# yaricom/Plastic-UNet

Hardware: AMD Instinct MI355X
Metric: training images/sec (128x128, bs=32 per GPU) (higher is better)
Workload: dtype f32; 1 GPU; C2: UNetp depth 5 base_ch 64, oja rule, 1x128x128, fwd+BCE+bwd+Adam; global_batch=32, per_gpu_batch=32, img=128, parallelism=single, step_launch=eager

## Files before the change

### include/plastic_unet.h

```cpp
#ifndef PLASTIC_UNET_H
#define PLASTIC_UNET_H

#include <stddef.h>
#include <stdint.h>

#ifdef __cplusplus
extern "C" {
#endif

#define PU_ABI_VERSION 3

typedef enum {
    PU_OK = 0,
    PU_ERR_INVALID = -1,
    PU_ERR_UNSUPPORTED = -2,
    PU_ERR_LAUNCH = -3,
    PU_ERR_WORKSPACE = -4
} pu_status;

int pu_abi_version(void);
const char* pu_last_error(void);
const char* pu_build_id(void);
int pu_device_info(int device, int* num_cu, int* clock_khz, long long* hbm_bytes);

enum { PU_EPI_RELU = 1, PU_EPI_ACCUM = 2, PU_EPI_SHUFFLE2 = 4, PU_EPI_RESID = 8, PU_CONV_NO_HALO = 16,
       PU_CONV_HALO_V1 = 32, PU_CONV_NO_SMALLX6 = 64, PU_CONV_HALO_DMA = 128, PU_EPI_OUT_BF16 = 256 };

typedef struct {
    int batch;
    int in_h, in_w;
    int out_h, out_w;
    int kh, kw, stride, pad;
    const float* src0; int c0;
    const float* src1; int c1;
    const float* weight; int k_pad; int cgroup;
    int n;
    const float* bias;
    float* dst0; int n0;
    float* dst1;
    const float* mask0;
    const float* mask1;
    int flags;
    void* workspace; size_t ws_bytes;
    const float* resid;
    int shuf_h, shuf_w, shuf_off;
    const void* weight6;
    const void* wino;
    const float* chan_scale; int chan_scale_ld;
} pu_conv_args;

int pu_conv_igemm(const pu_conv_args* a, void* stream);
typedef struct {
    const float* w;
    void* out;
    int cout, cin;
    int dgrad;
} pu_wino_job;
size_t pu_wino_bytes(int n, int c);
int pu_pack_wino(const pu_wino_job* jobs, int n_jobs, void* stream);
int pu_split_weight6(const float* packed, void* out, int n, int k_pad, void* stream);
size_t pu_conv_igemm_workspace_bytes(const pu_conv_args* a);
int pu_conv_igemm_tile(const pu_conv_args* a, int* bm, int* bn, int* mode, int* ksplit);

typedef struct {
    int batch;
    int in_h, in_w;
    int out_h, out_w;
    int kh, kw, stride, pad;
    const float* rows; int n;
    const float* src0; int c0;
    const float* src1; int c1;
    int bias_mode;
    float* dweight;
    float* dbias;
    int accumulate;
    int math;
} pu_wgrad_args;

size_t pu_wgrad_workspace_bytes(const pu_wgrad_args* a);
// ... 175 lines not shown
```

### plastic-unet_amd/csrc/igemm.hip

```cpp
#include "conv_common.h"
#include <type_traits>

namespace pu {


constexpr int IG_BK = 16;
constexpr int IG_LDS = IG_BK + 4;

enum { LOAD_CHUNK16 = 0, LOAD_VEC4 = 1, LOAD_SCALAR = 2 };


template <int MODE>
__device__ __forceinline__ f32x4 load_a4(const IgemmParams& p, int pb, int hb, int wb, int k) {
    f32x4 v = {0.f, 0.f, 0.f, 0.f};
    if (MODE == LOAD_SCALAR) {
#pragma unroll
        for (int e = 0; e < 4; ++e) {
            int ke = k + e;
            if (ke < p.K) {
                int tap = fdiv(ke, p.dC);
                int c = ke - tap * p.C;
                int r = fdiv(tap, p.dKw);
                int s = tap - r * p.kw;
                int hi = hb + r, wi = wb + s;
// ... 882 lines not shown
                xb[i] = *reinterpret_cast<const f32x4*>(a + (a_row0 + i * 32) * 16 + pos1);
            }
#pragma unroll
            for (int pl = 0; pl < 3; ++pl)
#pragma unroll
                for (int j = 0; j < FN; ++j)
                    fw[pl][j] = *reinterpret_cast<const bf16x8_t*>(wp + ((pl * 2 + lh) * BN + b_row0 + j * 32) * 4);
#pragma unroll
            for (int i = 0; i < FM; ++i) {
                bf16x8_t xh, xm, xl;
                split3_pairs(xa[i], xb[i], xh, xm, xl);
#pragma unroll
                for (int j = 0; j < FN; ++j) {
                    f32x16 c = acc[i][j];
                    c = __builtin_amdgcn_mfma_f32_32x32x16_bf16(fw[1][j], xm, c, 0, 0, 0);
                    c = __builtin_amdgcn_mfma_f32_32x32x16_bf16(fw[2][j], xh, c, 0, 0, 0);
                    c = __builtin_amdgcn_mfma_f32_32x32x16_bf16(fw[0][j], xl, c, 0, 0, 0);
                    c = __builtin_amdgcn_mfma_f32_32x32x16_bf16(fw[1][j], xh, c, 0, 0, 0);
                    c = __builtin_amdgcn_mfma_f32_32x32x16_bf16(fw[0][j], xm, c, 0, 0, 0);
                    c = __builtin_amdgcn_mfma_f32_32x32x16_bf16(fw[0][j], xh, c, 0, 0, 0);
                    acc[i][j] = c;
                }
                if (i == 0) {
                    if constexpr (u + 2 < SPG) issue(g, std::integral_constant<int, u + 2>{});
                    else issue(g + 1, std::integral_constant<int, u + 2 - SPG>{});
                }
            }
        });
    }
    asm volatile("s_waitcnt vmcnt(0)" ::: "memory");
    if (p.ksplit == 1) {
        epilogue<BM, BN, WM, WN, true>(p, acc, m_blk, n_blk, wm, wn, lr, lh);
        return;
    }
    float* part = p.part + (long long)kz * p.M * p.N;
#pragma unroll
    for (int i = 0; i < FM; ++i) {
        const int m = m_blk + wm * (BM / WM) + i * 32 + lr;
        if (m >= p.M) continue;
#pragma unroll
        for (int j = 0; j < FN; ++j)
#pragma unroll
            for (int q = 0; q < 4; ++q) {
                const int n = n_blk + wn * (BN / WN) + j * 32 + 8 * q + 4 * lh;
                if (n >= p.N) continue;
                f32x4 v;
#pragma unroll
                for (int e = 0; e < 4; ++e) v[e] = acc[i][j][4 * q + e];
                *reinterpret_cast<f32x4*>(part + (long long)m * p.N + n) = v;
            }
    }
}

__global__ void split_weight6_kernel(const float* __restrict__ w, __bf16* __restrict__ out, int n, int k_pad) {
#pragma clang fp contract(off)
    const long long total = (long long)n * k_pad;
    for (long long idx = blockIdx.x * 256LL + threadIdx.x; idx < total; idx += (long long)gridDim.x * 256) {
        const int row = (int)(idx / k_pad);
        const int k = (int)(idx - (long long)row * k_pad);
        const float x = w[idx];
        const __bf16 a = (__bf16)x;
        const float r = x - (float)a;
        const __bf16 b = (__bf16)r;
        const __bf16 c = (__bf16)(r - (float)b);
        const int t = k >> 4, half = (k >> 3) & 1, e = k & 7;
        const __bf16 v[3] = {a, b, c};
#pragma unroll
        for (int pl = 0; pl < 3; ++pl)
            out[(((long long)t * 6 + pl * 2 + half) * n + row) * 8 + e] = v[pl];
    }
}

__global__ __launch_bounds__(256) void igemm_splitk_epilogue_kernel(const IgemmParams p) {
    const int nq = p.N >> 2;
    const long long idx = (long long)blockIdx.x * 256 + threadIdx.x;
    if (idx >= (long long)p.M * nq) return;
    const int m = (int)(idx / nq);
    const int n = (int)(idx - (long long)m * nq) * 4;
    const long long mn = (long long)p.M * p.N;
    const float* src = p.part + (long long)m * p.N + n;
    f32x4 v = *reinterpret_cast<const f32x4*>(src);
    for (int z = 1; z < p.ksplit; ++z) v += *reinterpret_cast<const f32x4*>(src + z * mn);
    epi_store4(p, epi_row(p, m), n, v);
}

constexpr int SC_TH = 16, SC_TW = 32;

template <int C, int N, int KP = (9 * C + 15) / 16 * 16>
__global__ __launch_bounds__(256) void smallconv_kernel(const IgemmParams p) {
    constexpr int HH = SC_TH + 2, HWD = SC_TW + 2;
    constexpr int CP = (C + 3) & ~3;
    __shared__ __attribute__((aligned(16))) float tile[HH * HWD * CP];
    const int tiles_w = (p.Wo + SC_TW - 1) / SC_TW;
    const int tiles_h = (p.Ho + SC_TH - 1) / SC_TH;
    int blk = blockIdx.x;
    const int txi = blk % tiles_w;
    blk /= tiles_w;
    const int tyi = blk % tiles_h;
    const int b = blk / tiles_h;
    const int y0 = tyi * SC_TH - 1, x0 = txi * SC_TW - 1;
    const long long img = (long long)b * p.Hi * p.Wi;

    if (C % 4 == 0 && p.c0 % 4 == 0) {
        constexpr int Q = C / 4 > 0 ? C / 4 : 1;
        constexpr int NE = HH * HWD * Q;
        constexpr int PT = (NE + 255) / 256;
// ... 154 lines not shown
            typedef __bf16 bf16x4_t __attribute__((ext_vector_type(4)));
            bf16x4_t o;
#pragma unroll
            for (int e = 0; e < 4; ++e) o[e] = (__bf16)v[e];
            *reinterpret_cast<bf16x4_t*>(reinterpret_cast<__bf16*>(p.dst0) + (long long)m * N + 4 * lane_c) = o;
        } else if (plain) {
            if (p.bias) v += bias4;
            if (p.flags & PU_EPI_RELU) {
#pragma unroll
                for (int e = 0; e < 4; ++e) v[e] = fmaxf(v[e], 0.f);
            }
            *reinterpret_cast<f32x4*>(p.dst0 + (long long)m * N + 4 * lane_c) = v;
        } else {
            epi_store4(p, epi_row(p, m), 4 * lane_c, v);
        }
    }
}

template <int BM, int BN, int WM, int WN>
static void launch_mode(int mode, const IgemmParams& p, dim3 grid, hipStream_t s) {
    switch (mode) {
        case LOAD_CHUNK16: hipLaunchKernelGGL((igemm_kernel<BM, BN, WM, WN, LOAD_CHUNK16>), grid, dim3(256), 0, s, p); break;
        case LOAD_VEC4: hipLaunchKernelGGL((igemm_kernel<BM, BN, WM, WN, LOAD_VEC4>), grid, dim3(256), 0, s, p); break;
        default: hipLaunchKernelGGL((igemm_kernel<BM, BN, WM, WN, LOAD_SCALAR>), grid, dim3(256), 0, s, p); break;
    }
}

static int choose_mode(int c0, int c1) {
    if (c0 % 16 == 0 && c1 % 16 == 0) return LOAD_CHUNK16;
    if (c0 % 4 == 0 && c1 % 4 == 0) return LOAD_VEC4;
    return LOAD_SCALAR;
}

static bool vec_epilogue(const pu_conv_args* a) {
    const bool shuffle = a->flags & PU_EPI_SHUFFLE2;
    const int n0 = shuffle ? a->n : a->n0;
    const uintptr_t al = (uintptr_t)a->dst0 | (uintptr_t)a->dst1 | (uintptr_t)a->mask0 | (uintptr_t)a->mask1 |
                         (uintptr_t)a->bias | ((a->flags & PU_EPI_RESID) ? (uintptr_t)a->resid : 0);
    return (a->n % 4 == 0) && (n0 % 4 == 0) && (al & 15) == 0 && (!shuffle || (a->n / 4) % 4 == 0);
}

static bool uses_x6(const pu_conv_args* a);
static bool lean_ok(const pu_conv_args* a) {
    if (!uses_x6(a)) return false;
    const int C = a->c0 + a->c1;
    if (a->kh != 3 || a->kw != 3 || !(a->cgroup == 16 || a->cgroup == 32)) return false;
    if (a->c1 != 0 && a->c1 != a->c0) return false;
    if (a->k_pad != 9 * C) return false;
    const long long shift = (long long)a->pad * a->in_w + a->pad;
    if (((long long)a->batch * a->in_h * a->in_w + shift) * a->c0 * 4 >= (1LL << 31)) return false;
    if ((long long)a->k_pad * a->n * 12 >= (1LL << 31)) return false;
    return true;
}
static void plan_tiles(const pu_conv_args* a, long long M, int* bm, int* bn, int* ksplit, int* t_per) {
    const int N = a->n;
    const int T = a->k_pad / IG_BK;
    if (!uses_x6(a)) {
        choose_tile(M, N, bm, bn);
        *ksplit = 1;
        *t_per = T;
        if (choose_mode(a->c0, a->c1) == LOAD_CHUNK16 && vec_epilogue(a))
            plan_split(a->k_pad, IG_BK, 8, M, N, *bm, *bn, ksplit, t_per);
        return;
    }
    int target = 512;
    if (N <= 32 && lean_ok(a)) {
        *bn = 32;
        *bm = blocks_for(M, N, 256, 32) >= 480 ? 256 : 128;
    } else if (N <= 64) {
        *bn = 64;
        *bm = blocks_for(M, N, 256, 64) >= 480 ? 256 : 128;
    } else if (a->k_pad >= 2048) {
        *bn = 128;
        *bm = 256;
        target = 256;
    } else {
        *bn = 128;
        *bm = 128;
    }
    *ksplit = 1;
    *t_per = T;
    const int tiles = blocks_for(M, N, *bm, *bn);
    if (tiles >= target - target / 16 || !vec_epilogue(a)) return;
    int ks = ceil_div(target, tiles);
    if (ks > T / 8) ks = T / 8;
    if (ks < 2) return;
    *t_per = ceil_div(T, ks);
    if (lean_ok(a)) {
        const int spg = 9 * (a->cgroup / 16);
        *t_per = ceil_div(*t_per, spg) * spg;
    }
    *ksplit = ceil_div(T, *t_per);
}

static bool conv1x1_small_ok(const pu_conv_args* a) {
    const int C = a->c0 + a->c1;
    return (C == 4 || C == 8) && (a->n == 8 || a->n == 16) && a->kh == 1 && a->kw == 1 && a->stride == 1 &&
           a->pad == 0 && a->in_h == a->out_h && a->in_w == a->out_w && !(a->flags & PU_EPI_SHUFFLE2) &&
           vec_epilogue(a) && a->c0 % 4 == 0 && a->c1 % 4 == 0 && (a->cgroup == 0 || a->cgroup >= C);
}

static bool small_conv_ok(const pu_conv_args* a) {
    const int C = a->c0 + a->c1;
    const bool cset = C == 1 || C == 4 || C == 8 || C == 12 || C == 16;
    const bool nset = a->n == 4 || a->n == 8 || a->n == 16;
    const bool nc = (a->n == 4) ? (C == 4 || C == 8 || C == 16) : true;
    return cset && nset && nc && a->kh == 3 && a->kw == 3 && a->stride == 1 && a->pad == 1 &&
           a->in_h == a->out_h && a->in_w == a->out_w && !(a->flags & PU_EPI_SHUFFLE2) && vec_epilogue(a) &&
           (a->cgroup == 0 || a->cgroup >= C) && (C == 1 || (a->c0 % 4 == 0 && a->c1 % 4 == 0)) &&
           a->k_pad == (9 * C + 15) / 16 * 16;
}

static bool stem_conv_ok(const pu_conv_args* a) {
    const int C = a->c0 + a->c1;
    return C == 1 && a->c1 == 0 && (a->n == 8 || a->n == 16 || a->n == 32 || a->n == 64) && a->kh == 3 && a->kw == 3 && a->stride == 1 &&
           a->pad == 1 && a->in_h == a->out_h && a->in_w == a->out_w && !(a->flags & PU_EPI_SHUFFLE2) &&
           vec_epilogue(a) && (a->cgroup == 0 || a->cgroup >= C);
}

static bool uses_x6(const pu_conv_args* a) {
    return a->weight6 && choose_mode(a->c0, a->c1) == LOAD_CHUNK16 && !small_conv_ok(a);
}

enum { CK_STEM, CK_1X1, CK_SMALLX6, CK_DIRECT, CK_WINO, CK_X6_LEAN, CK_X6, CK_DMA, CK_LOADER };
struct ConvPlan {
    int kind, bm, bn;
    int mode;
    int ksplit, t_per;
    size_t ws_bytes;
};

static ConvPlan plan_conv(const pu_conv_args* a, long long M) {
    ConvPlan pl;
    pl.bn = a->n;
    pl.ksplit = 1;
    pl.t_per = a->k_pad / IG_BK;
    pl.ws_bytes = 0;
    const bool vec = vec_epilogue(a);
    if (stem_conv_ok(a)) {
        pl.kind = CK_STEM;
        pl.mode = 5;
        pl.bm = ST_TH * ST_TW;
        return pl;
    }
    if (conv1x1_small_ok(a)) {
        pl.kind = CK_1X1;
        pl.mode = 3;
        pl.bm = 256;
        return pl;
    }
    if (smallx6_ok(a, vec)) {
        pl.kind = CK_SMALLX6;
        pl.mode = 7;
        pl.bm = a->stride == 2 ? 128 : a->kh == 2 ? 256 : 512;
        return pl;
    }
    if (small_conv_ok(a)) {
        pl.kind = CK_DIRECT;
        pl.mode = 3;
        pl.bm = SC_TH * SC_TW;
        return pl;
    }
    if (wino_ok(a, vec)) {
        pl.kind = CK_WINO;
        pl.mode = 6;
        pl.bn = wino_item_channels(a);
        pl.bm = pl.bn == 64 ? 256 : 128;
        pl.ws_bytes = wino_workspace_bytes(a);
        if (pl.ws_bytes) pl.ksplit = (int)(pl.ws_bytes / ((size_t)M * a->n * sizeof(float)));
    } else {
        plan_tiles(a, M, &pl.bm, &pl.bn, &pl.ksplit, &pl.t_per);
        const int loader = choose_mode(a->c0, a->c1);
        pl.kind = uses_x6(a) ? (lean_ok(a) ? CK_X6_LEAN : CK_X6) : loader == LOAD_CHUNK16 ? CK_DMA : CK_LOADER;
        pl.mode = uses_x6(a) ? 4 : loader;
        if (pl.ksplit > 1) pl.ws_bytes = (size_t)pl.ksplit * (size_t)M * (size_t)a->n * sizeof(float);
    }
    if (pl.ksplit > 1 && (!a->workspace || a->ws_bytes < pl.ws_bytes)) {
        pl.ksplit = 1;
        pl.t_per = a->k_pad / IG_BK;
    }
    return pl;
}

}

using namespace pu;

extern "C" int pu_conv_igemm(const pu_conv_args* a, void* stream) {
    PU_REQUIRE(a != nullptr, "pu_conv_igemm: null args");
    PU_REQUIRE(a->batch > 0 && a->in_h > 0 && a->in_w > 0 && a->out_h > 0 && a->out_w > 0,
               "pu_conv_igemm: bad grid %dx%dx%d -> %dx%d", a->batch, a->in_h, a->in_w, a->out_h, a->out_w);
    PU_REQUIRE(a->kh > 0 && a->kw > 0 && a->stride > 0 && a->pad >= 0, "pu_conv_igemm: bad taps");
    PU_REQUIRE(a->kh * a->kw <= 32, "pu_conv_igemm: at most 32 taps");
    PU_REQUIRE(a->src0 && a->c0 > 0, "pu_conv_igemm: src0 missing");
    PU_REQUIRE(a->c1 == 0 || a->src1, "pu_conv_igemm: src1 missing for c1=%d", a->c1);
    PU_REQUIRE(a->weight && a->dst0 && a->n > 0, "pu_conv_igemm: weight/dst0/n");
    const int C = a->c0 + a->c1;
    const int K = a->kh * a->kw * C;
    PU_REQUIRE(a->k_pad >= K && a->k_pad % IG_BK == 0, "pu_conv_igemm: k_pad %d must be >= %d and a multiple of 16", a->k_pad, K);
    const bool shuffle = a->flags & PU_EPI_SHUFFLE2;
    if (a->flags & PU_EPI_RESID) {
        PU_REQUIRE(a->resid && !shuffle && (a->n0 == a->n), "pu_conv_igemm: RESID needs resid, a single destination, no SHUFFLE2");
    }
    if (shuffle) {
        PU_REQUIRE(a->n % 4 == 0, "pu_conv_igemm: SHUFFLE2 needs n %% 4 == 0");
        PU_REQUIRE(a->shuf_off >= 0 && a->shuf_h >= 0 && a->shuf_w >= 0, "pu_conv_igemm: shuffle geometry");
    } else {
        PU_REQUIRE(a->n0 > 0 && a->n0 <= a->n, "pu_conv_igemm: n0 %d out of range", a->n0);
        PU_REQUIRE(a->n0 == a->n || a->dst1, "pu_conv_igemm: dst1 missing");
    }
    const long long M = (long long)a->batch * a->out_h * a->out_w;
    PU_REQUIRE(M < (1LL << 31) && (long long)a->batch * a->in_h * a->in_w < (1LL << 31), "pu_conv_igemm: too many pixels");

    IgemmParams p;
    p.M = (int)M; p.N = a->n; p.K = K; p.k_pad = a->k_pad;
    p.Hi = a->in_h; p.Wi = a->in_w; p.Ho = a->out_h; p.Wo = a->out_w;
    p.kh = a->kh; p.kw = a->kw; p.stride = a->stride; p.pad = a->pad;
    p.C = C; p.c0 = a->c0; p.c1 = a->c1;
    p.src0 = a->src0; p.src1 = a->src1; p.wt = a->weight; p.bias = a->bias;
    p.dst0 = a->dst0; p.dst1 = a->dst1; p.mask0 = a->mask0; p.mask1 = a->mask1;
    p.n0 = shuffle ? a->n : a->n0; p.flags = a->flags;
    p.resid = (a->flags & PU_EPI_RESID) ? a->resid : nullptr;
    p.shuf_h = a->shuf_h ? a->shuf_h : 2 * a->out_h;
    p.shuf_w = a->shuf_w ? a->shuf_w : 2 * a->out_w;
    p.shuf_off = a->shuf_off;
    p.dWo = make_fastdiv(a->out_w); p.dHo = make_fastdiv(a->out_h);
    p.dC = make_fastdiv(C); p.dKw = make_fastdiv(a->kw); p.dCo = make_fastdiv(shuffle ? a->n / 4 : 1);
    p.taps = a->kh * a->kw;
    p.dTaps = make_fastdiv(p.taps);
    p.cgroup = a->cgroup;
    p.vec_epi = vec_epilogue(a);
    p.in_pix = a->batch * a->in_h * a->in_w;
    p.cscale = a->chan_scale;
    p.cs_ld = a->chan_scale_ld ? a->chan_scale_ld : (shuffle ? a->n / 4 : a->n);
    p.dHW = make_fastdiv(a->out_h * a->out_w);
    if (a->chan_scale) {
        PU_REQUIRE(((uintptr_t)a->chan_scale & 15) == 0 && p.cs_ld % 4 == 0 && p.cs_ld >= (shuffle ? a->n / 4 : a->n),
                   "pu_conv_igemm: chan_scale must be 16-byte aligned with a row stride >= its channels and %% 4 == 0 (ld %d)", p.cs_ld);
    }

    const int mode = choose_mode(a->c0, a->c1);
    PU_REQUIRE(a->cgroup == 0 || a->cgroup == 16 || a->cgroup == 32, "pu_conv_igemm: cgroup %d", a->cgroup);
    PU_REQUIRE(a->cgroup == 0 || (mode == LOAD_CHUNK16 && a->c0 % a->cgroup == 0 && a->c1 % a->cgroup == 0),
               "pu_conv_igemm: cgroup %d needs channel counts (%d, %d) that are multiples of it", a->cgroup, a->c0, a->c1);
    if (mode != LOAD_SCALAR) {
        PU_REQUIRE(((uintptr_t)a->src0 & 15) == 0 && ((uintptr_t)a->src1 & 15) == 0,
                   "pu_conv_igemm: sources must be 16-byte aligned");
    }
    PU_REQUIRE(((uintptr_t)a->weight & 15) == 0, "pu_conv_igemm: weight must be 16-byte aligned");

    const bool out_bf16 = a->flags & PU_EPI_OUT_BF16;
    if (out_bf16) {
        PU_REQUIRE(stem_conv_ok(a) && !a->mask0 && !a->mask1 && !a->resid && !a->chan_scale && a->n0 == a->n &&
                       !(a->flags & (PU_EPI_ACCUM | PU_EPI_SHUFFLE2)) && ((uintptr_t)a->dst0 & 7) == 0,
                   "pu_conv_igemm: PU_EPI_OUT_BF16 is the single-channel stem conv only (c0 1, 3x3/s1/p1, n 8/16/32/64, "
                   "no mask/resid/accum/shuffle/chan_scale, 8-byte aligned dst0)");
    }
    const ConvPlan pl = plan_conv(a, M);
    if (pl.kind == CK_WINO || pl.kind == CK_X6_LEAN || pl.kind == CK_X6) {
        PU_REQUIRE(((uintptr_t)a->weight6 & 15) == 0, "pu_conv_igemm: weight6 must be 16-byte aligned");
    }
    hipStream_t s = as_stream(stream);
    const int N = a->n;
    const int bm = pl.bm, bn = pl.bn;
    p.ksplit = pl.ksplit;
    p.t_per = pl.t_per;
    p.part = (float*)a->workspace;
    p.gn = ceil_div(N, bn);
    const dim3 grid(ceil_div(M, bm) * p.gn * p.ksplit);
    const char* what = "pu_conv_igemm";
    switch (pl.kind) {
        case CK_STEM: {
            const dim3 sgrid((unsigned)(((a->out_w + ST_TW - 1) / ST_TW) * ((a->out_h + ST_TH - 1) / ST_TH) * a->batch));
            if (out_bf16) {
                if (N == 64) hipLaunchKernelGGL((stem_conv_kernel<64, true>), sgrid, dim3(256), 0, s, p);
                else if (N == 32) hipLaunchKernelGGL((stem_conv_kernel<32, true>), sgrid, dim3(256), 0, s, p);
                else if (N == 16) hipLaunchKernelGGL((stem_conv_kernel<16, true>), sgrid, dim3(256), 0, s, p);
                else hipLaunchKernelGGL((stem_conv_kernel<8, true>), sgrid, dim3(256), 0, s, p);
                what = "pu_conv_igemm (stem, bf16 out)";
                break;
            }
            if (N == 64) hipLaunchKernelGGL((stem_conv_kernel<64>), sgrid, dim3(256), 0, s, p);
            else if (N == 32) hipLaunchKernelGGL((stem_conv_kernel<32>), sgrid, dim3(256), 0, s, p);
            else if (N == 16) hipLaunchKernelGGL((stem_conv_kernel<16>), sgrid, dim3(256), 0, s, p);
            else hipLaunchKernelGGL((stem_conv_kernel<8>), sgrid, dim3(256), 0, s, p);
            what = "pu_conv_igemm (stem)";
            break;
        }
        case CK_1X1: {
            const dim3 g1((unsigned)(M / 256 + 1 < 8192 ? M / 256 + 1 : 8192));
            if (C == 4 && N == 8) hipLaunchKernelGGL((conv1x1_small_kernel<4, 8>), g1, dim3(256), 0, s, p);
            else if (C == 4) hipLaunchKernelGGL((conv1x1_small_kernel<4, 16>), g1, dim3(256), 0, s, p);
            else if (N == 8) hipLaunchKernelGGL((conv1x1_small_kernel<8, 8>), g1, dim3(256), 0, s, p);
            else hipLaunchKernelGGL((conv1x1_small_kernel<8, 16>), g1, dim3(256), 0, s, p);
            what = "pu_conv_igemm (1x1 small-channel)";
            break;
        }
        case CK_SMALLX6:
            return smallx6_launch(a, p, s);
        case CK_DIRECT: {
            const dim3 sgrid((unsigned)(((a->out_w + SC_TW - 1) / SC_TW) * ((a->out_h + SC_TH - 1) / SC_TH) * a->batch));
#define PU_SC(C_, N_) if (C == C_ && N == N_) hipLaunchKernelGGL((smallconv_kernel<C_, N_>), sgrid, dim3(256), 0, s, p)
            PU_SC(1, 8); else PU_SC(1, 16); else PU_SC(4, 8); else PU_SC(4, 16); else PU_SC(8, 8); else PU_SC(8, 16);
            else PU_SC(12, 8); else PU_SC(12, 16); else PU_SC(16, 8); else PU_SC(16, 16);
            else PU_SC(4, 4); else PU_SC(8, 4); else PU_SC(16, 4);
#undef PU_SC
            what = "pu_conv_igemm (small-channel)";
            break;
        }
        case CK_WINO:
            p.gn = N / 64;
            wino_launch(a, p, s);
            what = "pu_conv_igemm (winograd x6)";
            break;
        case CK_X6_LEAN: {
            p.wt = reinterpret_cast<const float*>(a->weight6);
            const int cg = a->cgroup / 16;
#define PU_XL(BM_, BN_, WM_, WN_, NW_)                                                                          \
    do {                                                                                                        \
        if (cg == 2) hipLaunchKernelGGL((igemm_x6_lean_kernel<BM_, BN_, WM_, WN_, NW_, 2>), grid, dim3(NW_ * 64), 0, s, p); \
        else hipLaunchKernelGGL((igemm_x6_lean_kernel<BM_, BN_, WM_, WN_, NW_, 1>), grid, dim3(NW_ * 64), 0, s, p); \
    } while (0)
            if (bm == 256 && bn == 128) PU_XL(256, 128, 8, 1, 8);
            else if (bm == 256 && bn == 64) PU_XL(256, 64, 8, 1, 8);
            else if (bm == 128 && bn == 128) PU_XL(128, 128, 4, 1, 4);
            else if (bm == 128 && bn == 64) PU_XL(128, 64, 2, 2, 4);
            else if (bm == 256) PU_XL(256, 32, 4, 1, 4);
            else PU_XL(128, 32, 4, 1, 4);
#undef PU_XL
            what = "pu_conv_igemm (x6 lean)";
            break;
        }
        case CK_X6:
            p.wt = reinterpret_cast<const float*>(a->weight6);
#define PU_X6(BM_, BN_, WM_, WN_) hipLaunchKernelGGL((igemm_x6_kernel<BM_, BN_, WM_, WN_>), grid, dim3(256), 0, s, p)
            if (bm == 256 && bn == 128)
                hipLaunchKernelGGL((igemm_x6_kernel<256, 128, 8, 1, 8>), grid, dim3(512), 0, s, p);
            else if (bm == 256) PU_X6(256, 64, 4, 1);
            else if (bm == 128 && bn == 128) PU_X6(128, 128, 4, 1);
            else PU_X6(128, 64, 2, 2);
#undef PU_X6
            break;
        case CK_DMA:
            if (bm == 256) hipLaunchKernelGGL((igemm_dma_kernel<256, 64, 4, 1, 3>), grid, dim3(256), 0, s, p);
            else if (bm == 128 && bn == 128) hipLaunchKernelGGL((igemm_dma_kernel<128, 128, 2, 2, 3>), grid, dim3(256), 0, s, p);
            else if (bm == 128) hipLaunchKernelGGL((igemm_dma_kernel<128, 64, 2, 2, 3>), grid, dim3(256), 0, s, p);
            else hipLaunchKernelGGL((igemm_dma_kernel<64, 64, 2, 2, 3>), grid, dim3(256), 0, s, p);
            break;
        default:
            if (bm == 256) launch_mode<256, 64, 4, 1>(pl.mode, p, grid, s);
            else if (bm == 128 && bn == 128) launch_mode<128, 128, 2, 2>(pl.mode, p, grid, s);
            else if (bm == 128) launch_mode<128, 64, 2, 2>(pl.mode, p, grid, s);
            else launch_mode<64, 64, 2, 2>(pl.mode, p, grid, s);
    }
    if (p.ksplit > 1) {
        const long long threads = M * (N / 4);
        hipLaunchKernelGGL(igemm_splitk_epilogue_kernel, dim3((unsigned)((threads + 255) / 256)), dim3(256), 0, s, p);
    }
    return check_launch(what);
}

extern "C" int pu_split_weight6(const float* packed, void* out, int n, int k_pad, void* stream) {
    PU_REQUIRE(packed && out && n > 0 && k_pad > 0 && k_pad % IG_BK == 0, "pu_split_weight6: bad args");
    const long long total = (long long)n * k_pad;
    long long blocks = (total + 255) / 256;
    if (blocks > 4096) blocks = 4096;
    hipLaunchKernelGGL(split_weight6_kernel, dim3((unsigned)blocks), dim3(256), 0, as_stream(stream), packed,
                       (__bf16*)out, n, k_pad);
    return check_launch("pu_split_weight6");
}

extern "C" size_t pu_conv_igemm_workspace_bytes(const pu_conv_args* a) {
    if (!a || a->batch <= 0 || a->out_h <= 0 || a->out_w <= 0 || a->n <= 0 || a->k_pad <= 0) return 0;
    return plan_conv(a, (long long)a->batch * a->out_h * a->out_w).ws_bytes;
}

extern "C" int pu_conv_igemm_tile(const pu_conv_args* a, int* bm, int* bn, int* mode, int* ksplit) {
    PU_REQUIRE(a && bm && bn && mode, "pu_conv_igemm_tile: null args");
    const ConvPlan pl = plan_conv(a, (long long)a->batch * a->out_h * a->out_w);
    *bm = pl.bm;
    *bn = pl.bn;
    *mode = pl.mode;
    if (ksplit) *ksplit = pl.ksplit;
    return PU_OK;
}
// ... 1 lines not shown
```

### plastic-unet_amd/punet/_lib.py

```python
import ctypes
import os

HERE = os.path.dirname(os.path.abspath(__file__))
LIB_PATH = os.environ.get("PLASTIC_UNET_LIB",
                          os.path.join(os.path.dirname(HERE), "lib", "libplastic_unet.so"))

c_int, c_ll, c_size, c_float, c_void_p = ctypes.c_int, ctypes.c_longlong, ctypes.c_size_t, ctypes.c_float, ctypes.c_void_p
c_double = ctypes.c_double
P = ctypes.c_void_p

(PU_EPI_RELU, PU_EPI_ACCUM, PU_EPI_SHUFFLE2, PU_EPI_RESID, PU_CONV_NO_HALO, PU_CONV_HALO_V1, PU_CONV_NO_SMALLX6,
 PU_CONV_HALO_DMA, PU_EPI_OUT_BF16) = 1, 2, 4, 8, 16, 32, 64, 128, 256
PU_PACK_CONV_FWD, PU_PACK_CONV_DGRAD, PU_PACK_CONVT_FWD, PU_PACK_CONVT_DGRAD, PU_PACK_CONVT3_FWD = 0, 1, 2, 3, 4
PU_RULE_HEBB, PU_RULE_OJA = 0, 1


ABI_VERSION = 3


class ConvArgs(ctypes.Structure):
    _fields_ = [("batch", c_int), ("in_h", c_int), ("in_w", c_int), ("out_h", c_int), ("out_w", c_int),
                ("kh", c_int), ("kw", c_int), ("stride", c_int), ("pad", c_int),
                ("src0", P), ("c0", c_int), ("src1", P), ("c1", c_int),
                ("weight", P), ("k_pad", c_int), ("cgroup", c_int), ("n", c_int), ("bias", P),
                ("dst0", P), ("n0", c_int), ("dst1", P), ("mask0", P), ("mask1", P), ("flags", c_int),
                ("workspace", P), ("ws_bytes", c_size),
                ("resid", P), ("shuf_h", c_int), ("shuf_w", c_int), ("shuf_off", c_int),
                ("weight6", P), ("wino", P), ("chan_scale", P), ("chan_scale_ld", c_int)]


class WgradArgs(ctypes.Structure):
    _fields_ = [("batch", c_int), ("in_h", c_int), ("in_w", c_int), ("out_h", c_int), ("out_w", c_int),
                ("kh", c_int), ("kw", c_int), ("stride", c_int), ("pad", c_int),
                ("rows", P), ("n", c_int), ("src0", P), ("c0", c_int), ("src1", P), ("c1", c_int),
                ("bias_mode", c_int), ("dweight", P), ("dbias", P), ("accumulate", c_int),
                ("math", c_int)]


class PlasticArgs(ctypes.Structure):
    _fields_ = [("batch", c_int), ("nbf", c_int), ("x", P), ("hebb", P), ("w", P), ("alpha", P), ("eta", P),
                ("y", P), ("hebb_out", P), ("rule", c_int)]


class PlasticHeadArgs(ctypes.Structure):
    _fields_ = [("batch", c_int), ("nbf", c_int), ("channels", c_int), ("feat", P), ("feat_bf16", c_int),
                ("out_w", P), ("out_b", P), ("hebb", P), ("w", P), ("alpha", P), ("eta", P), ("x", P), ("y", P),
                ("hebb_out", P), ("rule", c_int)]


class PlasticBwdArgs(ctypes.Structure):
    _fields_ = [("batch", c_int), ("nbf", c_int), ("x", P), ("hebb", P), ("w", P), ("alpha", P), ("y", P),
                ("dy", P), ("dx", P), ("dw", P), ("dalpha", P)]


class PlasticBwdTraceArgs(ctypes.Structure):
    _fields_ = [("batch", c_int), ("nbf", c_int), ("rule", c_int), ("x", P), ("hebb", P), ("w", P), ("alpha", P),
                ("eta", P), ("y", P), ("dy", P), ("dhebb_out", P), ("dx", P), ("dw", P), ("dalpha", P), ("dhebb", P),
                ("deta", P)]


class AdamTensor(ctypes.Structure):
    _fields_ = [("param", P), ("grad", P), ("exp_avg", P), ("exp_avg_sq", P), ("numel", c_ll)]


class WinoJob(ctypes.Structure):
# ... 111 lines not shown
```

### plastic-unet_amd/punet/kernels.py

```python
import ctypes
import os

import torch

from . import _lib
from ._lib import (ConvArgs, WgradArgs, PlasticArgs, PlasticHeadArgs, PlasticBwdArgs, PlasticBwdTraceArgs, AdamTensor,
                   PackJob, WinoJob, check,
                   PU_EPI_RELU, PU_EPI_ACCUM, PU_EPI_SHUFFLE2, PU_EPI_RESID, PU_CONV_NO_HALO, PU_CONV_HALO_V1,
                   PU_CONV_NO_SMALLX6, PU_EPI_OUT_BF16)

__all__ = ["KernelProfiler", "igemm", "wgrad", "pack_weight", "nchw_to_nhwc", "maxpool2_fwd", "maxpool2_bwd",
           "outconv_fwd", "outconv_bwd", "plastic_fwd", "trace_update", "plastic_bwd", "plastic_bwd_trace", "bce_fwd",
           "bce_bwd", "adam_multi", "pack_weights", "round16", "cgroup_for", "device_info", "lib"]


def lib():
    return _lib.load()


_PROF = None
_MODES = {0: "chunk16", 1: "vec4", 2: "scalar", 3: "direct", 4: "x6", 5: "stem", 6: "wino", 7: "x6s"}

_FP32_MATH = os.environ.get("PU_FP32_MATH", "split6")


_CONV_HALO = os.environ.get("PU_CONV_HALO", "1") != "0"


def set_conv_halo(on):
    global _CONV_HALO
    if isinstance(on, str) or on not in (0, 1):
        raise ValueError("set_conv_halo: 1 / True (halo and rows) or 0 / False (per-tap), not %r" % (on,))
    prev, _CONV_HALO = int(_CONV_HALO), bool(on)
    return prev


def _halo_flags():
    return 0 if _CONV_HALO else PU_CONV_NO_HALO


def fp32_math():
    return _FP32_MATH


_WINO = os.environ.get("PU_WINO", "1") != "0"


_SMALLX6 = os.environ.get("PU_SMALLX6", "1") != "0"


def set_smallx6(on):
    global _SMALLX6
    prev, _SMALLX6 = _SMALLX6, bool(on)
    return prev


def set_wino(on):
    global _WINO
    prev, _WINO = _WINO, bool(on)
    return prev


def wino_wanted(w, mode):
    if mode not in (0, 1) or w.dim() != 4 or w.shape[2:] != (3, 3) or _FP32_MATH != "split6":
        return False
    n, c = (w.shape[0], w.shape[1]) if mode == 0 else (w.shape[1], w.shape[0])
    return c % 32 == 0 and n % 64 == 0 and (c >= 128 or n <= 64 or n % 128 == 0)


def pack_wino(jobs):
    if not jobs:
        return
    arr = (WinoJob * len(jobs))()
    nbytes = 0.0
    for i, (w, out, dgrad) in enumerate(jobs):
        _req(w, "w")
        arr[i] = WinoJob(w.data_ptr(), out.data_ptr(), w.shape[0], w.shape[1], int(dgrad))
        nbytes += 4.0 * w.numel() + 2.0 * out.numel()
    with _Rec("pack_wino", nbytes=nbytes):
        check(lib().pu_pack_wino(arr, len(jobs), _stream()), "pu_pack_wino")


def set_fp32_math(mode):
    global _FP32_MATH
    if mode not in ("split6", "native"):
        raise ValueError("fp32 math must be 'split6' or 'native', got %r" % (mode,))
    prev, _FP32_MATH = _FP32_MATH, mode
    return prev


class KernelProfiler:

    def __init__(self):
        self.records = []

    def __enter__(self):
        global _PROF
        self._prev, _PROF = _PROF, self
        return self

    def __exit__(self, *exc):
# ... 47 lines not shown
    return torch.cuda.current_stream().cuda_stream


def round16(k):
    return (k + 15) // 16 * 16


def _req(t, name, dtype=torch.float32):
    if t is None:
        return
    if not t.is_cuda:
        raise RuntimeError("%s must be on the ROCm device (got %s); the plastic U-Net path has no CPU "
                           "fallback" % (name, t.device))
    if t.dtype != dtype:
        raise RuntimeError("%s must be %s (got %s)" % (name, dtype, t.dtype))
    if not t.is_contiguous():
        raise RuntimeError("%s must be contiguous" % name)


BF16 = torch.bfloat16


def _act_dtype(t):
    return BF16 if t.dtype == BF16 else torch.float32


def device_info(device=0):
    L = lib()
    cu, clk, mem = ctypes.c_int(), ctypes.c_int(), ctypes.c_longlong()
    check(L.pu_device_info(device, ctypes.byref(cu), ctypes.byref(clk), ctypes.byref(mem)), "pu_device_info")
    return cu.value, clk.value, mem.value


def cgroup_for(c0, c1=0):
    if c0 % 32 == 0 and c1 % 32 == 0:
        return 32
    if c0 % 16 == 0 and c1 % 16 == 0:
        return 16
    return 0


def igemm(*, batch, in_hw, out_hw, k, stride, pad, src0, c0, weight, k_pad, n, dst0, n0=None,
          src1=None, c1=0, bias=None, dst1=None, mask0=None, mask1=None, relu=False, accum=False,
          shuffle=False, cgroup=0, resid=None, shuf=(0, 0, 0), chan_scale=None):
    dt = _act_dtype(src0)
    out_bf16 = dt == torch.float32 and dst0 is not None and dst0.dtype == BF16
    for t, nm in ((src0, "src0"), (src1, "src1"), (weight, "weight"), (dst0, "dst0"),
                  (dst1, "dst1"), (mask0, "mask0"), (mask1, "mask1"), (resid, "resid")):
        _req(t, nm, BF16 if (out_bf16 and nm == "dst0") else dt)
    _req(bias, "bias")
    _req(chan_scale, "chan_scale")
    flags = (PU_EPI_RELU if relu else 0) | (PU_EPI_ACCUM if accum else 0) | (PU_EPI_SHUFFLE2 if shuffle else 0) \
        | (PU_EPI_RESID if resid is not None else 0) | _halo_flags() | (0 if _SMALLX6 else PU_CONV_NO_SMALLX6) \
        | (PU_EPI_OUT_BF16 if out_bf16 else 0)
    a = ConvArgs(batch, in_hw[0], in_hw[1], out_hw[0], out_hw[1], k, k, stride, pad,
                 _p(src0), c0, _p(src1), c1, _p(weight), k_pad, cgroup, n, _p(bias),
                 _p(dst0), n if n0 is None else n0, _p(dst1), _p(mask0), _p(mask1), flags, None, 0,
                 _p(resid), shuf[0], shuf[1], shuf[2])
    if chan_scale is not None:
        if chan_scale.dim() != 2 or chan_scale.shape[0] != batch:
            raise RuntimeError("chan_scale must be [batch, channels]")
        a.chan_scale, a.chan_scale_ld = chan_scale.data_ptr(), chan_scale.shape[1]
    w6 = getattr(weight, "_split6", None) if (dt != BF16 and _FP32_MATH == "split6") else None
    wn = getattr(weight, "_wino", None) if (w6 is not None and _WINO) else None
    if w6 is not None:
        a.weight6 = w6.data_ptr()
    if wn is not None:
        a.wino = wn.data_ptr()
        key = (batch, tuple(in_hw), tuple(out_hw), k, stride, pad, c0, c1, n, a.n0, k_pad, cgroup, flags,
               tuple(None if t is None else t.data_ptr() % 16
                     for t in (src0, src1, bias, dst0, dst1, mask0, mask1, resid, chan_scale, weight, w6, wn)))
        _ensure_direct(a, weight, key)
    elif getattr(weight, "_direct_ok", True) is False:
        _refresh_direct(weight)
    L = lib()
    if dt == BF16:
        _igemm_bf16(L, a, batch, out_hw, k, c0, c1, n, dst0)
        return
    nbytes = L.pu_conv_igemm_workspace_bytes(ctypes.byref(a))
    if nbytes:
        ws = torch.empty(nbytes // 4 + 1, dtype=torch.float32, device=dst0.device)
        a.workspace, a.ws_bytes = ws.data_ptr(), nbytes
    if _PROF is None:
        check(L.pu_conv_igemm(ctypes.byref(a), _stream()), "pu_conv_igemm")
        return
    bm, bn, mode, ks = ctypes.c_int(), ctypes.c_int(), ctypes.c_int(), ctypes.c_int()
    L.pu_conv_igemm_tile(ctypes.byref(a), ctypes.byref(bm), ctypes.byref(bn), ctypes.byref(mode), ctypes.byref(ks))
    M = batch * out_hw[0] * out_hw[1]
    tag = "igemm<%dx%d,%s%s>" % (bm.value, bn.value, _MODES[mode.value], ",k%d" % ks.value if ks.value > 1 else "")
    nb = 0.0
    if mode.value in (3, 5, 7):
        per = (c0 + c1) + n * (1 + int(accum) + int(resid is not None)) + n0_mask(n, n0, mask0, mask1)
        nb = 4.0 * M * per
    with _Rec(tag, flops=2.0 * M * n * k * k * (c0 + c1), nbytes=nb):
        check(L.pu_conv_igemm(ctypes.byref(a), _stream()), "pu_conv_igemm")


def n0_mask(n, n0, mask0, mask1):
    n0 = n if n0 is None else n0
    return (n0 if mask0 is not None else 0) + (n - n0 if mask1 is not None else 0)


def _igemm_bf16(L, a, batch, out_hw, k, c0, c1, n, dst0):
    nbytes = L.pu_conv_igemm_bf16_workspace_bytes(ctypes.byref(a))
    if nbytes:
        ws = torch.empty(nbytes // 4 + 1, dtype=torch.float32, device=dst0.device)
        a.workspace, a.ws_bytes = ws.data_ptr(), nbytes
# ... 449 lines not shown
```

Baseline: 4723 images/s.

## Add lean direct-to-LDS x6 kernel for 1x1 and 2x2-stride-2 convolutions

Adds a new split-bf16 (x6) implicit-GEMM kernel for pointwise 1x1 and 2x2 stride-2 convolutions. It uses buffer loads straight into LDS, a triple-buffered stage ring, and precomputed per-lane offsets. Before this, those shapes fell to the generic x6 kernel with its heavier loader. The aim is to cut address arithmetic and overlap global loads with MFMA work. The path is on by default and can be disabled by an environment variable or flag; it adds a new code path with its own tile-selection and bounds checks.

```diff
diff --git a/include/plastic_unet.h b/include/plastic_unet.h
--- a/include/plastic_unet.h
+++ b/include/plastic_unet.h
@@ -24,7 +24,8 @@
 int pu_device_info(int device, int* num_cu, int* clock_khz, long long* hbm_bytes);
 
 enum { PU_EPI_RELU = 1, PU_EPI_ACCUM = 2, PU_EPI_SHUFFLE2 = 4, PU_EPI_RESID = 8, PU_CONV_NO_HALO = 16,
-       PU_CONV_HALO_V1 = 32, PU_CONV_NO_SMALLX6 = 64, PU_CONV_HALO_DMA = 128, PU_EPI_OUT_BF16 = 256 };
+       PU_CONV_HALO_V1 = 32, PU_CONV_NO_SMALLX6 = 64, PU_CONV_HALO_DMA = 128, PU_EPI_OUT_BF16 = 256,
+       PU_CONV_NO_POINT_LEAN = 512 };
 
 typedef struct {
     int batch;
diff --git a/plastic-unet_amd/csrc/igemm.hip b/plastic-unet_amd/csrc/igemm.hip
--- a/plastic-unet_amd/csrc/igemm.hip
+++ b/plastic-unet_amd/csrc/igemm.hip
@@ -958,6 +958,181 @@
     }
 }
 
+template <int BM, int BN, int WM, int WN, int NW, int TAPS, int CG>
+__global__ __launch_bounds__(NW * 64) void igemm_x6_point_kernel(const IgemmParams p) {
+    constexpr int FM = BM / WM / 32;
+    constexpr int FN = BN / WN / 32;
+    constexpr int A_LD = BM / (16 * NW);
+    constexpr int W_TOT = 6 * BN / 64;
+    constexpr int W_LD = (W_TOT + NW - 1) / NW;
+    constexpr bool SINK = (W_TOT % NW) != 0;
+    constexpr int G = A_LD + W_LD;
+    constexpr int A_FL = BM * 16;
+    constexpr int W_FL = BN * 6 * 4;
+    constexpr int STAGE = A_FL + W_FL;
+    static_assert(WM * WN == NW && A_LD >= 1 && (TAPS == 1 || TAPS == 4) && (CG == 1 || CG == 2), "point tile");
+
+    __shared__ __attribute__((aligned(16))) float lds[3 * STAGE + (SINK ? 256 : 0)];
+
+    const int tid = threadIdx.x;
+    const int lane = tid & 63;
+    const int wave = __builtin_amdgcn_readfirstlane(tid >> 6);
+    const int wm = wave % WM, wn = wave / WM;
+    const int lr = lane & 31, lh = lane >> 5;
+    int tile = xcd_remap(blockIdx.x, gridDim.x);
+    const int kz = tile / (gridDim.x / p.ksplit);
+    tile -= kz * (gridDim.x / p.ksplit);
+    const int mb = tile / p.gn;
+    const int m_blk = mb * BM;
+    const int n_blk = (tile - mb * p.gn) * BN;
+
+    const int cs = p.c0;
+    const unsigned a_bytes = (unsigned)((long long)p.in_pix * cs * 4);
+    const unsigned w_bytes = (unsigned)((long long)p.k_pad * p.N * 6);
+
+    const int lq = lane >> 2;
+    const int kc = (lane & 3) ^ ((lane >> 4) & 3);
+    unsigned vo[A_LD];
+#pragma unroll
+    for (int j = 0; j < A_LD; ++j) {
+        const int m = m_blk + wave * (BM / NW) + 16 * j + lq;
+        unsigned o = LEAN_OOB;
+        if (m < p.M) {
+            int pix = m;
+            if constexpr (TAPS == 4) {
+                const int t = fdiv(m, p.dWo);
+                const int wo = m - t * p.Wo;
+                const int b = fdiv(t, p.dHo);
+                const int ho = t - b * p.Ho;
+                pix = (b * p.Hi + 2 * ho) * p.Wi + 2 * wo;
+            }
+            o = (unsigned)pix * (unsigned)(cs * 4) + kc * 16;
+        }
+        vo[j] = o;
+    }
+    unsigned wv[W_LD];
+#pragma unroll
+    for (int j = 0; j < W_LD; ++j) {
+        const int I = wave + NW * j;
+        const int e = I * 64 + lane;
+        const int q = e / BN, row = e - q * BN;
+        const int n = n_blk + row;
+        wv[j] = (I < W_TOT && n < p.N) ? (unsigned)((q * p.N + n) * 16) : LEAN_OOB;
+    }
+    const unsigned w_stage = (unsigned)p.N * 96u;
+    const unsigned row_bytes = (unsigned)(p.Wi * cs * 4), pix_bytes = (unsigned)(cs * 4);
+
+    const int t0 = kz * p.t_per;
+    const int T = min(p.k_pad / IG_BK - t0, p.t_per);
+
+    auto issue = [&](int tl, auto sc) {
+        constexpr int slot = decltype(sc)::value;
+        const bool live = tl < T;
+        const unsigned t = (unsigned)(t0 + tl);
+        unsigned soff;
+        if constexpr (TAPS == 1) {
+            soff = t * 64u;
+        } else {
+            const unsigned tg = t / CG, h = t % CG;
+            const unsigned g = tg >> 2, tap = tg & 3;
+            soff = (tap >> 1) * row_bytes + (tap & 1) * pix_bytes + (g * (16 * CG) + h * 16) * 4u;
+        }
+        float* a_slot = lds + slot * STAGE;
+        const unsigned abytes = live ? a_bytes : 0u;
+#pragma unroll
+        for (int j = 0; j < A_LD; ++j)
+            lean_load(p.src0, abytes, a_slot + (wave * (BM / NW) + 16 * j) * 16, vo[j], soff);
+        const unsigned wbytes = live ? w_bytes : 0u;
+        const unsigned wsoff = t * w_stage;
+        float* w_slot = a_slot + A_FL;
+#pragma unroll
+        for (int j = 0; j < W_LD; ++j) {
+            const int I = wave + NW * j;
+            float* dst = (!SINK || I < W_TOT) ? w_slot + I * 256 : lds + 3 * STAGE;
+            lean_load(p.wt, wbytes, dst, wv[j], wsoff);
+        }
+    };
+
+    f32x16 acc[FM][FN];
+#pragma unroll
+    for (int i = 0; i < FM; ++i)
+#pragma unroll
+        for (int j = 0; j < FN; ++j)
+#pragma unroll
+            for (int r = 0; r < 16; ++r) acc[i][j][r] = 0.f;
+
+    const int a_row0 = wm * (BM / WM) + lr;
+    const int b_row0 = wn * (BN / WN) + lr;
+    const int swz = (lr >> 2) & 3;
+    const int pos0 = ((2 * lh) ^ swz) * 4, pos1 = ((2 * lh + 1) ^ swz) * 4;
+
+    issue(0, std::integral_constant<int, 0>{});
+    issue(1, std::integral_constant<int, 1>{});
+    for (int ts = 0; ts < T; ts += 3) {
+        static_for<3>([&](auto uc) {
+            constexpr int u = decltype(uc)::value;
+            if (ts + u < T) {
+                asm volatile("s_waitcnt vmcnt(%0)" ::"n"(G) : "memory");
+                __builtin_amdgcn_s_barrier();
+                asm volatile("" ::: "memory");
+                const float* a = lds + u * STAGE;
+                const float* wp = a + A_FL;
+                f32x4 xa[FM], xb[FM];
+                bf16x8_t fw[3][FN];
+#pragma unroll
+                for (int i = 0; i < FM; ++i) {
+                    xa[i] = *reinterpret_cast<const f32x4*>(a + (a_row0 + i * 32) * 16 + pos0);
+                    xb[i] = *reinterpret_cast<const f32x4*>(a + (a_row0 + i * 32) * 16 + pos1);
+                }
+#pragma unroll
+                for (int pl = 0; pl < 3; ++pl)
+#pragma unroll
+                    for (int j = 0; j < FN; ++j)
+                        fw[pl][j] = *reinterpret_cast<const bf16x8_t*>(wp + ((pl * 2 + lh) * BN + b_row0 + j * 32) * 4);
+#pragma unroll
+                for (int i = 0; i < FM; ++i) {
+                    bf16x8_t xh, xm, xl;
+                    split3_pairs(xa[i], xb[i], xh, xm, xl);
+#pragma unroll
+                    for (int j = 0; j < FN; ++j) {
+                        f32x16 c = acc[i][j];
+                        c = __builtin_amdgcn_mfma_f32_32x32x16_bf16(fw[1][j], xm, c, 0, 0, 0);
+                        c = __builtin_amdgcn_mfma_f32_32x32x16_bf16(fw[2][j], xh, c, 0, 0, 0);
+                        c = __builtin_amdgcn_mfma_f32_32x32x16_bf16(fw[0][j], xl, c, 0, 0, 0);
+                        c = __builtin_amdgcn_mfma_f32_32x32x16_bf16(fw[1][j], xh, c, 0, 0, 0);
+                        c = __builtin_amdgcn_mfma_f32_32x32x16_bf16(fw[0][j], xm, c, 0, 0, 0);
+                        c = __builtin_amdgcn_mfma_f32_32x32x16_bf16(fw[0][j], xh, c, 0, 0, 0);
+                        acc[i][j] = c;
+                    }
+                    if (i == 0) issue(ts + u + 2, std::integral_constant<int, (u + 2) % 3>{});
+                }
+            }
+        });
+    }
+    asm volatile("s_waitcnt vmcnt(0)" ::: "memory");
+    if (p.ksplit == 1) {
+        epilogue<BM, BN, WM, WN, true>(p, acc, m_blk, n_blk, wm, wn, lr, lh);
+        return;
+    }
+    float* part = p.part + (long long)kz * p.M * p.N;
+#pragma unroll
+    for (int i = 0; i < FM; ++i) {
+        const int m = m_blk + wm * (BM / WM) + i * 32 + lr;
+        if (m >= p.M) continue;
+#pragma unroll
+        for (int j = 0; j < FN; ++j)
+#pragma unroll
+            for (int q = 0; q < 4; ++q) {
+                const int n = n_blk + wn * (BN / WN) + j * 32 + 8 * q + 4 * lh;
+                if (n >= p.N) continue;
+                f32x4 v;
+#pragma unroll
+                for (int e = 0; e < 4; ++e) v[e] = acc[i][j][4 * q + e];
+                *reinterpret_cast<f32x4*>(part + (long long)m * p.N + n) = v;
+            }
+    }
+}
+
 __global__ void split_weight6_kernel(const float* __restrict__ w, __bf16* __restrict__ out, int n, int k_pad) {
 #pragma clang fp contract(off)
     const long long total = (long long)n * k_pad;
@@ -1218,6 +1393,20 @@
     if ((long long)a->k_pad * a->n * 12 >= (1LL << 31)) return false;
     return true;
 }
+static bool point_lean_ok(const pu_conv_args* a) {
+    if (!uses_x6(a) || (a->flags & PU_CONV_NO_POINT_LEAN)) return false;
+    const bool g1 = a->kh == 1 && a->kw == 1 && a->stride == 1 && a->pad == 0 && a->in_h == a->out_h &&
+                    a->in_w == a->out_w && a->cgroup == 0;
+    const bool g4 = a->kh == 2 && a->kw == 2 && a->stride == 2 && a->pad == 0 && a->in_h == 2 * a->out_h &&
+                    a->in_w == 2 * a->out_w && (a->cgroup == 16 || a->cgroup == 32) && a->c0 % a->cgroup == 0;
+    if (!g1 && !g4) return false;
+    if (a->c1 != 0 || a->k_pad != a->kh * a->kw * a->c0 || !vec_epilogue(a)) return false;
+    const long long lim = 1LL << 31;
+    if ((long long)a->batch * a->in_h * a->in_w * a->c0 * 4 >= lim) return false;
+    if ((long long)a->k_pad * a->n * 6 >= lim) return false;
+    if ((long long)a->batch * a->out_h * a->out_w * a->n * 4 >= lim) return false;
+    return true;
+}
 static void plan_tiles(const pu_conv_args* a, long long M, int* bm, int* bn, int* ksplit, int* t_per) {
     const int N = a->n;
     const int T = a->k_pad / IG_BK;
@@ -1288,7 +1477,7 @@
     return a->weight6 && choose_mode(a->c0, a->c1) == LOAD_CHUNK16 && !small_conv_ok(a);
 }
 
-enum { CK_STEM, CK_1X1, CK_SMALLX6, CK_DIRECT, CK_WINO, CK_X6_LEAN, CK_X6, CK_DMA, CK_LOADER };
+enum { CK_STEM, CK_1X1, CK_SMALLX6, CK_DIRECT, CK_WINO, CK_X6_LEAN, CK_X6_POINT, CK_X6, CK_DMA, CK_LOADER };
 struct ConvPlan {
     int kind, bm, bn;
     int mode;
@@ -1337,7 +1526,8 @@
     } else {
         plan_tiles(a, M, &pl.bm, &pl.bn, &pl.ksplit, &pl.t_per);
         const int loader = choose_mode(a->c0, a->c1);
-        pl.kind = uses_x6(a) ? (lean_ok(a) ? CK_X6_LEAN : CK_X6) : loader == LOAD_CHUNK16 ? CK_DMA : CK_LOADER;
+        pl.kind = uses_x6(a) ? (lean_ok(a) ? CK_X6_LEAN : point_lean_ok(a) ? CK_X6_POINT : CK_X6)
+                             : loader == LOAD_CHUNK16 ? CK_DMA : CK_LOADER;
         pl.mode = uses_x6(a) ? 4 : loader;
         if (pl.ksplit > 1) pl.ws_bytes = (size_t)pl.ksplit * (size_t)M * (size_t)a->n * sizeof(float);
     }
@@ -1423,7 +1613,7 @@
                    "no mask/resid/accum/shuffle/chan_scale, 8-byte aligned dst0)");
     }
     const ConvPlan pl = plan_conv(a, M);
-    if (pl.kind == CK_WINO || pl.kind == CK_X6_LEAN || pl.kind == CK_X6) {
+    if (pl.kind == CK_WINO || pl.kind == CK_X6_LEAN || pl.kind == CK_X6_POINT || pl.kind == CK_X6) {
         PU_REQUIRE(((uintptr_t)a->weight6 & 15) == 0, "pu_conv_igemm: weight6 must be 16-byte aligned");
     }
     hipStream_t s = as_stream(stream);
@@ -1497,6 +1687,23 @@
             what = "pu_conv_igemm (x6 lean)";
             break;
         }
+        case CK_X6_POINT: {
+            p.wt = reinterpret_cast<const float*>(a->weight6);
+            const int taps = a->kh * a->kw, cg = a->cgroup == 32 ? 2 : 1;
+#define PU_XP(BM_, BN_, WM_, WN_, NW_)                                                                          \
+    do {                                                                                                        \
+        if (taps == 1) hipLaunchKernelGGL((igemm_x6_point_kernel<BM_, BN_, WM_, WN_, NW_, 1, 1>), grid, dim3(NW_ * 64), 0, s, p); \
+        else if (cg == 2) hipLaunchKernelGGL((igemm_x6_point_kernel<BM_, BN_, WM_, WN_, NW_, 4, 2>), grid, dim3(NW_ * 64), 0, s, p); \
+        else hipLaunchKernelGGL((igemm_x6_point_kernel<BM_, BN_, WM_, WN_, NW_, 4, 1>), grid, dim3(NW_ * 64), 0, s, p); \
+    } while (0)
+            if (bm == 256 && bn == 128) PU_XP(256, 128, 8, 1, 8);
+            else if (bm == 256) PU_XP(256, 64, 4, 1, 4);
+            else if (bm == 128 && bn == 128) PU_XP(128, 128, 4, 1, 4);
+            else PU_XP(128, 64, 2, 2, 4);
+#undef PU_XP
+            what = "pu_conv_igemm (x6 point)";
+            break;
+        }
         case CK_X6:
             p.wt = reinterpret_cast<const float*>(a->weight6);
 #define PU_X6(BM_, BN_, WM_, WN_) hipLaunchKernelGGL((igemm_x6_kernel<BM_, BN_, WM_, WN_>), grid, dim3(256), 0, s, p)
diff --git a/plastic-unet_amd/punet/_lib.py b/plastic-unet_amd/punet/_lib.py
--- a/plastic-unet_amd/punet/_lib.py
+++ b/plastic-unet_amd/punet/_lib.py
@@ -10,7 +10,7 @@
 P = ctypes.c_void_p
 
 (PU_EPI_RELU, PU_EPI_ACCUM, PU_EPI_SHUFFLE2, PU_EPI_RESID, PU_CONV_NO_HALO, PU_CONV_HALO_V1, PU_CONV_NO_SMALLX6,
- PU_CONV_HALO_DMA, PU_EPI_OUT_BF16) = 1, 2, 4, 8, 16, 32, 64, 128, 256
+ PU_CONV_HALO_DMA, PU_EPI_OUT_BF16, PU_CONV_NO_POINT_LEAN) = 1, 2, 4, 8, 16, 32, 64, 128, 256, 512
 PU_PACK_CONV_FWD, PU_PACK_CONV_DGRAD, PU_PACK_CONVT_FWD, PU_PACK_CONVT_DGRAD, PU_PACK_CONVT3_FWD = 0, 1, 2, 3, 4
 PU_RULE_HEBB, PU_RULE_OJA = 0, 1
 
diff --git a/plastic-unet_amd/punet/kernels.py b/plastic-unet_amd/punet/kernels.py
--- a/plastic-unet_amd/punet/kernels.py
+++ b/plastic-unet_amd/punet/kernels.py
@@ -7,7 +7,7 @@
 from ._lib import (ConvArgs, WgradArgs, PlasticArgs, PlasticHeadArgs, PlasticBwdArgs, PlasticBwdTraceArgs, AdamTensor,
                    PackJob, WinoJob, check,
                    PU_EPI_RELU, PU_EPI_ACCUM, PU_EPI_SHUFFLE2, PU_EPI_RESID, PU_CONV_NO_HALO, PU_CONV_HALO_V1,
-                   PU_CONV_NO_SMALLX6, PU_EPI_OUT_BF16)
+                   PU_CONV_NO_SMALLX6, PU_EPI_OUT_BF16, PU_CONV_NO_POINT_LEAN)
 
 __all__ = ["KernelProfiler", "igemm", "wgrad", "pack_weight", "nchw_to_nhwc", "maxpool2_fwd", "maxpool2_bwd",
            "outconv_fwd", "outconv_bwd", "plastic_fwd", "trace_update", "plastic_bwd", "plastic_bwd_trace", "bce_fwd",
@@ -47,6 +47,15 @@
 
 
 _SMALLX6 = os.environ.get("PU_SMALLX6", "1") != "0"
+
+
+_POINT_LEAN = os.environ.get("PU_POINT_LEAN", "1") != "0"
+
+
+def set_point_lean(on):
+    global _POINT_LEAN
+    prev, _POINT_LEAN = _POINT_LEAN, bool(on)
+    return prev
 
 
 def set_smallx6(on):
@@ -200,7 +209,7 @@
     _req(chan_scale, "chan_scale")
     flags = (PU_EPI_RELU if relu else 0) | (PU_EPI_ACCUM if accum else 0) | (PU_EPI_SHUFFLE2 if shuffle else 0) \
         | (PU_EPI_RESID if resid is not None else 0) | _halo_flags() | (0 if _SMALLX6 else PU_CONV_NO_SMALLX6) \
-        | (PU_EPI_OUT_BF16 if out_bf16 else 0)
+        | (PU_EPI_OUT_BF16 if out_bf16 else 0) | (0 if _POINT_LEAN else PU_CONV_NO_POINT_LEAN)
     a = ConvArgs(batch, in_hw[0], in_hw[1], out_hw[0], out_hw[1], k, k, stride, pad,
                  _p(src0), c0, _p(src1), c1, _p(weight), k_pad, cgroup, n, _p(bias),
                  _p(dst0), n if n0 is None else n0, _p(dst1), _p(mask0), _p(mask1), flags, None, 0,
```

New measurement: 4599 images/s. -2.6%, worse.
